# Polochon-street/bliss-rs

Hardware: AMD Instinct MI355X
Metric: songs/sec (3-min 22 050 Hz f32) at 1/2/4/8 GPU; HBM GB/s vs roofline (higher is better)
Workload: dtype f32; 1 GPU; configs[1]: batch of 1024 synthetic 3969000-sample (3-min) white-noise f32 PCM buffers per GPU, full 23-feature descriptor set (FeaturesVersion 2); songs_per_gpu=1024, songs_total=1024, features=23, parallelism=single GPU

## Files before the change

bliss-rs_amd/csrc/kernels_chroma.hip:

```cpp
#include <float.h>
#include <stdlib.h>

#include <type_traits>

#include "device_utils.hpp"
#include "fft_r16.hpp"
#include "internal.hpp"

namespace bg {

typedef double double4_t __attribute__((ext_vector_type(4)));

__device__ __forceinline__ double tuning_of_slot(int slot) {
    return slot >= N_TUNING ? 0.0 : (-50.0 + (100.0 * 0.01 * (double)slot)) / 100.0;
}

__global__ __launch_bounds__(256) void chroma_bank_kernel(double* __restrict__ bank) {
#pragma clang fp contract(off)
    const int slot = blockIdx.y;
    const int k = blockIdx.x * 256 + threadIdx.x;
    if (k >= BANK_PITCH) return;
    double* out = bank + (size_t)slot * BANK_ROWS * BANK_PITCH;
    if (k >= CBINS) {
        for (int r = 0; r < BANK_ROWS; r++) out[(size_t)r * BANK_PITCH + k] = 0.0;
        return;
    }
    const double tuning = tuning_of_slot(slot);
    const double ncf = 12.0, nc2 = 6.0;
    const double step = 22050.0 / 8192.0;
    const double a440 = 440.0 * pow(2.0, tuning / 12.0);
    auto fbin = [&](int i) { return log2((0.0 + step * (double)i) / (a440 / 16.0)) * ncf; };
    const double fb1 = fbin(1);
    const double fb = (k == 0) ? fb1 - 1.5 * ncf : fbin(k);
    const double fbn = fbin(k + 1);
    double bw = fbn - fb;
    if (bw <= 1.0) bw = 1.0;
    double w[12], l2 = 0.0;
    for (int c = 0; c < 12; c++) {
        double d = -(double)c + fb;
        d = fmod(d + nc2 + 10.0 * ncf, ncf) - nc2;
        d = d / bw;
        w[c] = exp(-0.5 * (2.0 * d) * (2.0 * d));
        l2 += w[c] * w[c];
    }
    l2 = sqrt(l2);
    if (l2 < DBL_MIN) l2 = 1.0;
    const double y = (fb / ncf - 5.0) / 2.0;
    const double g = exp(-0.5 * (y * y));
    for (int r = 0; r < BANK_ROWS; r++) {
        double v = 0.0;
        if (r < 12) v = (w[(r + 3) % 12] / l2) * g;
        out[(size_t)r * BANK_PITCH + k] = v;
    }
}

void launch_chroma_bank(double* bank, hipStream_t st) {
    hipLaunchKernelGGL(chroma_bank_kernel, dim3((BANK_PITCH + 255) / 256, N_TUNING + 1), dim3(256), 0, st, bank);
}

__device__ __forceinline__ bool pip_is_peak(float sb, float se, float sa, double ref) {
    return (sa <= se) && (sb < se) && ((double)se > ref);
}

__device__ __forceinline__ void wave_append(bool is_peak, int c, uint16_t* list, uint32_t* count) {
    const uint64_t mask = __ballot(is_peak);
    if (mask == 0) return;
    const uint32_t lane = (uint32_t)lane_id();
    uint32_t base = 0;
    if (lane == 0) base = atomicAdd(count, (uint32_t)__popcll(mask));
    base = __shfl(base, 0, WAVE);
    if (is_peak) list[base + (uint32_t)__popcll(mask & ((1ull << lane) - 1ull))] = (uint16_t)c;
}

__device__ __forceinline__ bool pip_peak_core(float sb, float se, float sa, double ref, int c, double* mag_out,
                                              double* pitch_out) {
#pragma clang fp contract(off)
    if (!(sa <= se && sb < se)) return false;
    const double before = (double)sb, elem = (double)se, after = (double)sa;
    if (!(elem > ref)) return false;
    const double avg = 0.5 * (after - before);
    double shift = 2.0 * elem - after - before;
    if (fabs(shift) < DBL_MIN) shift += 1.0;
    shift = avg / shift;
    const double pitch = ((double)c + shift) * 22050.0 / 8192.0;
    if (!(pitch > 0.0)) return false;
    *mag_out = elem + 0.5 * avg * shift;
    *pitch_out = pitch;
    return true;
}

__device__ __forceinline__ bool pip_peak_mag(float sb, float se, float sa, double ref, int c, double* mag_out) {
    double pitch;
    return pip_peak_core(sb, se, sa, ref, c, mag_out, &pitch);
}

__device__ __forceinline__ int pitch_bin(double pitch) {
#pragma clang fp contract(off)
    double x = log2(pitch / (440.0 / 16.0));
    x = 12.0 * x;
    x = x - trunc(x);
    if (x >= 0.5) x -= 1.0;
    const double q = (x - -0.5) / 0.01;
    int idx = (q > 0.0) ? (int)q : 0;
    if (idx > N_TUNING - 1) idx = N_TUNING - 1;
    return idx;
}

__device__ __forceinline__ uint32_t coarse_bin(double mag) {
    const uint32_t b = __float_as_uint((float)mag) >> COARSE_SHIFT;
    return b < (uint32_t)H1_BINS ? b : (uint32_t)H1_BINS - 1;
}

__device__ __forceinline__ float ref_floor_f32(double ref) {
    float f = (float)ref;
    if ((double)f > ref) f = __uint_as_float(__float_as_uint(f) - 1u);
    return f;
}

__device__ __forceinline__ uint32_t peak_coarse_bin(float sb, float se, float sa, double ref, int c) {
    const float avg = 0.5f * (sa - sb);
    const float den = (2.0f * se - sa) - sb;
    const float shift = avg * __builtin_amdgcn_rcpf(den);
    const uint32_t bits = __float_as_uint(se + (0.5f * avg) * shift), low = bits & COARSE_LOW_MASK;
    if (se >= 1e-30f && low >= 16u && low <= COARSE_LOW_MASK - 16u) {
        const uint32_t b = bits >> COARSE_SHIFT;
        return b < (uint32_t)H1_BINS ? b : (uint32_t)H1_BINS - 1;
    }
    double mag;
    pip_peak_mag(sb, se, sa, ref, c, &mag);
    return coarse_bin(mag);
}

constexpr float PITCH_GUARD = 0.008f, PITCH_FLAT_LIMIT = 0.00390625f;
__device__ __forceinline__ int peak_pitch_bin_f32(float sb, float se, float sa, int c) {
    const float avg = 0.5f * (sa - sb);
    const float den = (2.0f * se - sa) - sb;
    if (!(se >= 1e-30f) || den < se * PITCH_FLAT_LIMIT) return -1;
    const float shift = avg * __builtin_amdgcn_rcpf(den);
    float x = 12.0f * (__builtin_amdgcn_logf((float)c + shift) + -3.3528687f);
    x = x - truncf(x);
    if (x >= 0.5f) x -= 1.0f;
    const float q = (x + 0.5f) * 100.0f;
    const float fl = floorf(q), fr = q - fl;
    if (fr < PITCH_GUARD || fr > 1.0f - PITCH_GUARD) return -1;
    const int idx = (int)fl;
    return idx < 0 ? 0 : (idx > N_TUNING - 1 ? N_TUNING - 1 : idx);
}

__device__ __attribute__((noinline)) uint32_t coarse_bin_exact(float sb, float se, float sa, double ref, int c) {
    double mag;
    pip_peak_mag(sb, se, sa, ref, c, &mag);
    return coarse_bin(mag);
}

__device__ __forceinline__ uint32_t peak_classify(float sb, float se, float sa, double ref, int c, int* pitch_bin_out) {
    const float avg = 0.5f * (sa - sb);
    const float den = (2.0f * se - sa) - sb;
    const float shift = avg * __builtin_amdgcn_rcpf(den);
    const bool normal = se >= 1e-30f;
    int pb = -1;
    if (normal && !(den < se * PITCH_FLAT_LIMIT)) {
        float x = 12.0f * (__builtin_amdgcn_logf((float)c + shift) + -3.3528687f);
        x = x - truncf(x);
        if (x >= 0.5f) x -= 1.0f;
        const float q = (x + 0.5f) * 100.0f;
        const float fl = floorf(q), fr = q - fl;
        if (!(fr < PITCH_GUARD || fr > 1.0f - PITCH_GUARD)) {
            const int idx = (int)fl;
            pb = idx < 0 ? 0 : (idx > N_TUNING - 1 ? N_TUNING - 1 : idx);
        }
    }
    *pitch_bin_out = pb;
    const uint32_t bits = __float_as_uint(se + (0.5f * avg) * shift), low = bits & COARSE_LOW_MASK;
    if (normal && low >= 16u && low <= COARSE_LOW_MASK - 16u) {
        const uint32_t b = bits >> COARSE_SHIFT;
        return b < (uint32_t)H1_BINS ? b : (uint32_t)H1_BINS - 1;
    }
    return coarse_bin_exact(sb, se, sa, ref, c);
}

__device__ __forceinline__ uint32_t peak_record(uint32_t coarse, int pitch_bin_or_neg, int c) {
    return (coarse << 18) | ((uint32_t)(pitch_bin_or_neg + 1) << 11) | (uint32_t)c;
}

constexpr int STFT_FRAMES_PER_WG = STFT_TILE;
constexpr int STFT_GROUP = 4;
constexpr int LHIST_BINS = 512;
constexpr int EX1_PITCH = 257;
constexpr int EX2_PITCH = 272;
constexpr int STFT_LDS = 16 * EX2_PITCH;
constexpr int MAGS_TOP = 2 * 4096;

__device__ constexpr float CONST_COS32[8] = {1.0f, 0.98078528040323044f, 0.92387953251128674f, 0.83146961230254524f,
                                             0.70710678118654752f, 0.55557023301960222f, 0.38268343236508977f, 0.19509032201612827f};
__device__ constexpr float CONST_SIN32[8] = {0.0f, 0.19509032201612827f, 0.38268343236508977f, 0.55557023301960222f,
                                             0.70710678118654752f, 0.83146961230254524f, 0.92387953251128674f, 0.98078528040323044f};

typedef unsigned int u32x2_t __attribute__((ext_vector_type(2)));
typedef unsigned int u32x4_t __attribute__((ext_vector_type(4)));
__device__ __forceinline__ f2 buf_load_f2(__amdgpu_buffer_rsrc_t r, uint32_t voff, uint32_t soff) {
    const u32x2_t v = __builtin_amdgcn_raw_buffer_load_b64(r, voff, soff, 0);
    return mk(__uint_as_float(v.x), __uint_as_float(v.y));
}

__device__ __forceinline__ long reflect_index(long p, long n) {
    if (p < 0) p = -p;
    else if (p >= n) p = 2 * n - 2 - p;
    return p;
}

#ifndef TRACE
#define TRACE_DECL
#define TRACE_INIT() do {} while (0)
#define TRACE_START() do {} while (0)
#define TRACE(k) do {} while (0)
#define TRACE_FLUSH() do {} while (0)
#endif

constexpr int STFT_LDS_N = 16 * EX2_PITCH;
constexpr int EXN1_PITCH = 260;
template <bool LOADWIN, bool HALVES>
__global__ __launch_bounds__(256, (LOADWIN && HALVES) ? 5 : 4) void stft8192_kernel(const float* __restrict__ pcm,
                                                       const SongDesc* __restrict__ songs, uint32_t n_songs,
                                                       const uint32_t* __restrict__ pfx_c,
                                                       const float* __restrict__ hann,
                                                       const float2* __restrict__ tw,
                                                       float* __restrict__ spec,
                                                       float* __restrict__ frame_max, uint32_t* __restrict__ h1,
                                                       uint32_t* __restrict__ peak_rec, uint32_t* __restrict__ peak_cnt,
                                                       uint32_t n_tiles) {
    constexpr bool NARROW = HALVES;
    __shared__ __attribute__((aligned(16))) float lds_raw[NARROW ? STFT_LDS_N : 2 * STFT_LDS];
    f2* const lds = reinterpret_cast<f2*>(lds_raw);
    float* const ldsf = lds_raw;
    constexpr int MAGS_TOP_W = NARROW ? 4096 : MAGS_TOP;
    __shared__ float red[4];
    __shared__ uint32_t lhist[LHIST_BINS];
    __shared__ uint32_t lhist_base;
    __shared__ uint16_t peak_list[PIP_MAX_PER_FRAME + 2];
    __shared__ uint32_t peak_count;
    __shared__ __attribute__((aligned(16))) f2 tw256[256];
    TRACE_DECL
    TRACE_INIT();
    {
        const float2 a = tw[32 * (((threadIdx.x >> 4) * (threadIdx.x & 15)) & 255)];
        tw256[threadIdx.x] = mk(a.x, a.y);
    }
    const uint32_t bx = blockIdx.x;
    const uint32_t wg = (bx & ~31u) | ((bx & 7u) << 2) | ((bx >> 3) & 3u);
    if (wg >= n_tiles) return;
    const uint32_t s = find_segment(pfx_c, n_songs, wg);
    const SongDesc sd = songs[s];
    const uint32_t tile = wg - pfx_c[s];
    const uint32_t f_first = (tile >> 2) * (uint32_t)(STFT_GROUP * STFT_FRAMES_PER_WG) + (tile & 3u);
    const float* __restrict__ x = pcm + sd.pcm_off;
    const int t = threadIdx.x;
    const long n = (long)sd.n;
    const int lo4 = t & 15, hi4 = t >> 4;

    const __amdgpu_buffer_rsrc_t r_hann = __builtin_amdgcn_make_buffer_rsrc((void*)hann, 0, W8192 * 4, 0x00020000);


    const uint32_t t8 = 8u * (uint32_t)t;
    f2 win[16];
    if constexpr (!LOADWIN) {
#pragma unroll
        for (int n1 = 0; n1 < 16; n1++) win[n1] = buf_load_f2(r_hann, t8, 2048u * n1);
    }
    f2 c_p2, c_sp;
    {
        const float2 a = tw[2 * hi4 * lo4], b = tw[t];
        c_p2 = mk(a.x, a.y);
        c_sp = mk(b.x, b.y);
        asm volatile("" : "+v"(c_p2), "+v"(c_sp));
    }
    uint32_t* hist = h1 + (size_t)s * H1_BINS;
    for (int i = t; i < LHIST_BINS; i += 256) lhist[i] = 0;
    bool have_base = false;
    __syncthreads();

    auto tw_at = [&](int m, int k) -> f2 {
        typedef float f4 __attribute__((ext_vector_type(4)));
        const f4 pair = reinterpret_cast<const f4*>(tw256)[8 * m + (k >> 1)];
        return (k & 1) ? mk(pair.z, pair.w) : mk(pair.x, pair.y);
    };
    auto load_window = [&]() {
        if constexpr (LOADWIN) {
#pragma unroll
            for (int n1 = 0; n1 < 16; n1++) win[n1] = buf_load_f2(r_hann, t8, 2048u * n1);
        }
    };
    auto load_frame = [&](uint32_t f, f2 (&xr)[16]) {
        const long w0 = (long)f * HOP_C - W8192 / 2;
        if (w0 + W8192 / 2 > n) {
#pragma unroll
            for (int n1 = 0; n1 < 16; n1++) xr[n1] = mk(0.0f, 0.0f);
        } else if (w0 >= 0 && w0 + W8192 <= n) {
            const __amdgpu_buffer_rsrc_t r_x = __builtin_amdgcn_make_buffer_rsrc((void*)(x + w0), 0, W8192 * 4, 0x00020000);
#pragma unroll
            for (int n1 = 0; n1 < 16; n1++) xr[n1] = buf_load_f2(r_x, t8, 2048u * n1);
        } else {
            const int before = w0 < 0 ? (int)(-w0) : 0;
            const long rel_l = n - w0;
            const int rel = rel_l > 0x3fffffffL ? 0x3fffffff : (int)rel_l;
            const float* __restrict__ xw = x + w0;
#pragma unroll
            for (int n1 = 0; n1 < 16; n1++) {
                int q0 = 2 * (256 * n1 + t), q1 = q0 + 1;
                q0 = q0 < before ? 2 * before - q0 : (q0 >= rel ? 2 * rel - 2 - q0 : q0);
                q1 = q1 < before ? 2 * before - q1 : (q1 >= rel ? 2 * rel - 2 - q1 : q1);
                xr[n1] = mk(xw[q0], xw[q1]);
            }
        }
    };

    f2 v[16];
    if (f_first < sd.n_c) {
        load_frame(f_first, v);
        load_window();
#pragma unroll
        for (int n1 = 0; n1 < 16; n1++) v[n1] = v[n1] * win[n1];
    }
    TRACE_START();
#pragma unroll 1
    for (int fi = 0; fi < STFT_FRAMES_PER_WG; fi++) {
        const uint32_t f = f_first + (uint32_t)(STFT_GROUP * fi);
        if (f >= sd.n_c) break;
        radix16(v);
#pragma unroll
        for (int k1 = 1; k1 < 16; k1++)
            v[R16(k1)] = cmul_pk(v[R16(k1)], tw_at(hi4, k1));
        if constexpr (NARROW) {
            f2 u[16];
#pragma unroll
            for (int k1 = 0; k1 < 16; k1++) ldsf[k1 * EXN1_PITCH + t] = v[R16(k1)].x;
            __syncthreads();
#pragma unroll
            for (int m1 = 0; m1 < 16; m1++) u[m1].x = ldsf[lo4 * EXN1_PITCH + 16 * m1 + hi4];
            __syncthreads();
#pragma unroll
            for (int k1 = 0; k1 < 16; k1++) ldsf[k1 * EXN1_PITCH + t] = v[R16(k1)].y;
            __syncthreads();
#pragma unroll
            for (int m1 = 0; m1 < 16; m1++) u[m1].y = ldsf[lo4 * EXN1_PITCH + 16 * m1 + hi4];
#pragma unroll
            for (int m1 = 0; m1 < 16; m1++) v[m1] = u[m1];
        } else {
#pragma unroll
        for (int k1 = 0; k1 < 16; k1++) lds[k1 * EX1_PITCH + t] = v[R16(k1)];
        TRACE(0);
        __syncthreads();
        TRACE(1);
#pragma unroll
        for (int m1 = 0; m1 < 16; m1++) v[m1] = lds[lo4 * EX1_PITCH + 16 * m1 + hi4];
        }
        radix16(v);
        v[R16(0)] = cmul_pk(v[R16(0)], c_p2);
#pragma unroll
        for (int j1 = 1; j1 < 16; j1++) v[R16(j1)] = cmul_pk(v[R16(j1)], cmul_pk(tw_at(hi4, j1), c_p2));
        TRACE(2);
        __syncthreads();
        TRACE(3);
        if constexpr (NARROW) {
            f2 u[16];
#pragma unroll
            for (int j1 = 0; j1 < 16; j1++) ldsf[j1 * EX2_PITCH + t] = v[R16(j1)].x;
            __syncthreads();
#pragma unroll
            for (int m2 = 0; m2 < 16; m2++) u[m2].x = ldsf[hi4 * EX2_PITCH + 16 * m2 + lo4];
            __syncthreads();
#pragma unroll
            for (int j1 = 0; j1 < 16; j1++) ldsf[j1 * EX2_PITCH + t] = v[R16(j1)].y;
            __syncthreads();
#pragma unroll
            for (int m2 = 0; m2 < 16; m2++) u[m2].y = ldsf[hi4 * EX2_PITCH + 16 * m2 + lo4];
#pragma unroll
            for (int m2 = 0; m2 < 16; m2++) v[m2] = u[m2];
        } else {
#pragma unroll
        for (int j1 = 0; j1 < 16; j1++) lds[j1 * EX2_PITCH + t] = v[R16(j1)];
        TRACE(4);
        __syncthreads();
        TRACE(5);
#pragma unroll
        for (int m2 = 0; m2 < 16; m2++) v[m2] = lds[hi4 * EX2_PITCH + 16 * m2 + lo4];
        }
        radix16(v);
        TRACE(6);
        __syncthreads();
        TRACE(7);
        constexpr int ZOFF = NARROW ? 2048 : 0;
#pragma unroll
        for (int j2 = 8; j2 < 16; j2++) lds[t + 256 * j2 - ZOFF] = v[R16(j2)];
        TRACE(8);
        __syncthreads();
        TRACE(9);
        float m_lo[8], m_hi[8], m_mid = 0.0f;
        float mx = 0.0f;
#pragma unroll
        for (int j = 0; j < 8; j++) {
            const float CJ = CONST_COS32[j], SJ = CONST_SIN32[j];
            const int k = t + 256 * j;
            float sq_k, sq_m;
            const f2 w = j == 0 ? c_sp : cmul_pk_s(c_sp, mk(CJ, -SJ));
            const f2 zm = lds[(k == 0 ? 2048 : 4096 - k) - ZOFF];
            split_pair_sq(v[R16(j)], (j == 0 && t == 0) ? v[R16(0)] : zm, w, sq_k, sq_m);
            m_lo[j] = mag_from_sq(sq_k);
            m_hi[j] = mag_from_sq(sq_m);
            mx = fmaxf(mx, fmaxf(m_lo[j], m_hi[j]));
        }
        if (t == 0) {
            m_mid = mag_from_sq(split_one_sq(v[R16(8)], v[R16(8)], mk(0.0f, -1.0f)));
            mx = fmaxf(mx, m_mid);
        }
        const bool has_next = fi + 1 < STFT_FRAMES_PER_WG && f + STFT_GROUP < sd.n_c;
        if (has_next) load_frame(f + STFT_GROUP, v);
        mx = wave_max_dpp(mx);
        if constexpr (NARROW) __syncthreads();
        float* mags = reinterpret_cast<float*>(lds);
        float* mags_top = mags + MAGS_TOP_W - 4096;
#pragma unroll
        for (int j = 0; j < 8; j++) {
            mags[t + 256 * j] = m_lo[j];
            if (j == 0 && t == 0) mags_top[4096] = m_hi[0];
            else mags[4096 - (t + 256 * j)] = m_hi[j];
        }
        if (t == 0) mags[2048] = m_mid;
        if (t >= 1 && t < CBINS_PAD - 4096) mags_top[4096 + t] = 0.0f;
        {
            int slot = t >> 6;
            asm volatile("" : "+v"(slot));
            if (lane_id() == 0) red[slot] = mx;
        }
        if (t == 0) peak_count = 0;
        TRACE(10);
        __syncthreads();
        TRACE(11);
        auto store_row = [&]() {
            const __amdgpu_buffer_rsrc_t r_row = __builtin_amdgcn_make_buffer_rsrc(
                (void*)(spec + (sd.c_off + f) * (size_t)CBINS_PAD), 0, CBINS_PAD * 4, 0x00020000);
            const u32x4_t* mags4 = reinterpret_cast<const u32x4_t*>(lds);
#pragma unroll
            for (int i = 0; i < 5; i++) {
                const int q = t + 256 * i;
                if (i < 4 || q < CBINS_PAD / 4) {
                    const u32x4_t val = i < 4 ? mags4[q] : mags4[q - 1024 + MAGS_TOP_W / 4];
                    __builtin_amdgcn_raw_buffer_store_b128(val, r_row, 16u * (uint32_t)q, 0, 2);
                }
            }
        };
        store_row();
        mx = fmaxf(fmaxf(red[0], red[1]), fmaxf(red[2], red[3]));
        if (t == 0) frame_max[sd.c_off + f] = mx;
        if (!have_base) {
            if (t == 0) {
                const uint32_t top = coarse_bin((double)mx);
                lhist_base = top > (uint32_t)(LHIST_BINS * 3 / 4) ? top - (uint32_t)(LHIST_BINS * 3 / 4) : 0u;
            }
            have_base = true;
            __syncthreads();
        }
        TRACE(12);
        const uint32_t lbase = lhist_base;
        __builtin_amdgcn_s_setprio(2);
        const double ref = 0.1 * (double)mx;
        const float thr = ref_floor_f32(ref);
        {
            uint32_t hits = 0;
#pragma unroll
            for (int h = 0; h < 2; h++) {
                float sb3[3], se3[3], sa3[3];
#pragma unroll
                for (int q = 0; q < 3; q++) {
                    const int c = t + 256 * (3 * h + q);
                    sb3[q] = mags[c > 0 ? c - 1 : 0];
                    se3[q] = mags[c];
                    sa3[q] = mags[c + 1];
                }
#pragma unroll
                for (int q = 0; q < 3; q++) {
                    const int j = 3 * h + q, c = t + 256 * j;
                    const uint32_t in_range = (256 * j >= PIP_LO && 256 * j + 255 <= PIP_HI) ? 1u : (uint32_t)(c >= PIP_LO) & (uint32_t)(c <= PIP_HI);
                    const uint32_t pk = in_range & (uint32_t)(sa3[q] <= se3[q]) & (uint32_t)(sb3[q] < se3[q]) & (uint32_t)(se3[q] > thr);
                    hits |= pk << j;
                }
            }
            const uint32_t mine = (uint32_t)__popc(hits);
            const uint32_t incl = wave_scan_incl_u32_dpp(mine);
            uint32_t wbase = 0;
            if (lane_id() == 63) wbase = atomicAdd(&peak_count, incl);
            uint32_t pos = (uint32_t)__builtin_amdgcn_readlane((int)wbase, 63) + incl - mine;
#pragma unroll
            for (int j = 0; j < 6; j++)
                if ((hits >> j) & 1u) peak_list[pos++] = (uint16_t)(t + 256 * j);
            TRACE(13);
            __syncthreads();
            TRACE(14);
            const uint32_t n_peaks = peak_count;
            uint32_t* __restrict__ recs = peak_rec + (sd.c_off + f) * (size_t)PIP_MAX_PER_FRAME;
            if (t == 0) peak_cnt[sd.c_off + f] = n_peaks;
            int c_next = t < n_peaks ? (int)peak_list[t] : PIP_LO;
            for (uint32_t i = t; i < n_peaks; i += 256) {
                const int c = c_next;
                const float sb = mags[c - 1], se = mags[c], sa = mags[c + 1];
                c_next = i + 256 < n_peaks ? (int)peak_list[i + 256] : PIP_LO;
                int pb;
                const uint32_t b = peak_classify(sb, se, sa, ref, c, &pb), rel = b - lbase;
                recs[i] = peak_record(b, pb, c);
                if (rel < (uint32_t)LHIST_BINS) atomicAdd(&lhist[rel], 1u);
                else atomicAdd(&hist[b], 1u);
            }
        }
        __builtin_amdgcn_s_setprio(0);
        if (has_next) {
            load_window();
#pragma unroll
            for (int n1 = 0; n1 < 16; n1++) v[n1] = v[n1] * win[n1];
        }
        TRACE(15);
        __syncthreads();
        TRACE(16);
    }
    TRACE_FLUSH();
    if (have_base) {
        const uint32_t lbase = lhist_base;
        for (int i = t; i < LHIST_BINS; i += 256) {
            const uint32_t c = lhist[i];
            if (c) atomicAdd(&hist[lbase + i], c);
        }
    }
}

void launch_stft8192(const Batch& b, const Workspace& w, const DeviceTables& t, hipStream_t st, int shape) {
    if (b.tiles_c == 0) return;
    auto k = stft8192_kernel<false, false>;
    if (shape == 1) k = stft8192_kernel<true, true>;
    else if (shape == 2) k = stft8192_kernel<true, false>;
    else if (shape == 3) k = stft8192_kernel<false, true>;
    hipLaunchKernelGGL(k, dim3((b.tiles_c + 31u) & ~31u), dim3(256), 0, st,
                       b.pcm, b.songs, b.n_songs, b.pfx_c, t.hann8192, t.tw8192, w.spec, w.frame_max, w.h1, w.peak_rec, w.peak_cnt,
                       b.tiles_c);
}

__global__ __launch_bounds__(256) void tune_select_kernel(const SongDesc* __restrict__ songs,
                                                          const uint32_t* __restrict__ h1,
                                                          TuningState* __restrict__ tuning,
                                                          uint32_t* __restrict__ cand_cursor, uint32_t cand_pool,
                                                          uint32_t first_song) {
    __shared__ uint32_t wsum[4];
    __shared__ uint32_t s_total, s_blo, s_bhi;
    const uint32_t s = blockIdx.x + first_song;
    const int tid = threadIdx.x;
    TuningState* ts = tuning + s;
    auto no_peaks = [&]() {
        if (tid == 0) {
            ts->n_peaks = 0; ts->tuning_idx = -1; ts->n_cand = 0; ts->b_lo = 1; ts->b_hi = 0; ts->below = 0;
            ts->cand_off = 0; ts->cand_cap = 0;
        }
    };
    if (!songs[s].ok) { no_peaks(); return; }
    const uint32_t* hist = h1 + (size_t)s * H1_BINS;
    constexpr int PER = H1_BINS / 256;
    uint32_t local[PER], sum = 0;
#pragma unroll
    for (int i = 0; i < PER; i++) { local[i] = hist[tid * PER + i]; sum += local[i]; }
    const uint32_t incl = wave_scan_incl_u32(sum);
    if (lane_id() == 63) wsum[wave_id()] = incl;
    __syncthreads();
    uint32_t base = 0;
    for (int w = 0; w < wave_id(); w++) base += wsum[w];
    if (tid == 255) s_total = base + incl;
    __syncthreads();
    const uint32_t total = s_total;
    uint32_t before = base + incl - sum;
    if (total == 0) { no_peaks(); return; }
    const uint32_t r_lo = (total - 1) / 2, r_hi = total - 1 - r_lo;
    if (tid == 0) { ts->n_peaks = total; ts->n_cand = 0; ts->tuning_idx = -1; }
#pragma unroll
    for (int i = 0; i < PER; i++) {
        const uint32_t c = local[i];
        if (c) {
            if (before <= r_lo && r_lo < before + c) { ts->b_lo = tid * PER + i; ts->below = before; s_blo = tid * PER + i; }
            if (before <= r_hi && r_hi < before + c) { ts->b_hi = tid * PER + i; s_bhi = tid * PER + i; }
        }
        before += c;
    }
    __syncthreads();
    const uint32_t blo = s_blo, bhi = s_bhi;
    uint32_t mine = 0;
#pragma unroll
    for (int i = 0; i < PER; i++) {
        const uint32_t bin = tid * PER + i;
        if (bin >= blo && bin <= bhi) mine += local[i];
    }
    mine = wave_sum(mine);
    if (lane_id() == 0) wsum[wave_id()] = mine;
    __syncthreads();
    if (tid == 0) {
        const uint32_t want = wsum[0] + wsum[1] + wsum[2] + wsum[3];
        const uint32_t off = atomicAdd(cand_cursor, want);
        if (off <= cand_pool && want <= cand_pool - off) {
            ts->cand_off = off;
            ts->cand_cap = want;
        } else {
            atomicSub(cand_cursor, want);
            ts->cand_off = 0;
            ts->cand_cap = 0;
        }
    }
}

void launch_tune_select(const Batch& b, const Workspace& w, hipStream_t st, const SongRange* r) {
    const uint32_t s0 = r ? r->s0 : 0, s1 = r ? r->s1 : b.n_songs;
    if (s1 <= s0) return;
    hipLaunchKernelGGL(tune_select_kernel, dim3(s1 - s0), dim3(256), 0, st, b.songs, w.h1, w.tuning, w.cand_cursor,
                       w.cand_cap, s0);
}

constexpr int P2_SLOW_CAP = 1024;
constexpr int P2_FRAMES_PER_WAVE = CH_TILE / 4;

__global__ __launch_bounds__(256) void tune_pass2_kernel(const SongDesc* __restrict__ songs, uint32_t n_songs,
                                                         const uint32_t* __restrict__ pfx_ct,
                                                         const float* __restrict__ spec,
                                                         const float* __restrict__ frame_max,
                                                         const uint32_t* __restrict__ peak_rec,
                                                         const uint32_t* __restrict__ peak_cnt,
                                                         TuningState* __restrict__ tuning,
                                                         uint32_t* __restrict__ hist100,
                                                         double* __restrict__ cand_mag,
                                                         uint8_t* __restrict__ cand_pb, uint32_t first_tile) {
    __shared__ uint32_t hist[N_TUNING];
    __shared__ uint32_t slow_list[4][P2_SLOW_CAP];
    const uint32_t bx = blockIdx.x + first_tile;
    const uint32_t s = find_segment(pfx_ct, n_songs, bx);
    const SongDesc sd = songs[s];
    const uint32_t tile = bx - pfx_ct[s];
    const int tid = threadIdx.x, lane = lane_id(), wave = wave_id();
    TuningState* ts = tuning + s;
    const uint32_t b_lo = ts->b_lo, b_hi = ts->b_hi;
    if (ts->n_peaks == 0) return;
    const uint32_t cand_off = ts->cand_off;
    const uint32_t cand_cap = ts->cand_cap;
    const bool pooled = cand_cap != 0;
    if (tid < N_TUNING) hist[tid] = 0;
    __syncthreads();
    uint32_t n_slow = 0;

    auto flush = [&]() {
        for (uint32_t i = lane; i < n_slow; i += WAVE) {
            const uint32_t e = slow_list[wave][i];
            const int c = (int)(e & 0xFFFFu);
            const uint32_t f = tile * CH_TILE + wave + 4 * (e >> 16);
            const float* row = spec + (sd.c_off + f) * (size_t)CBINS_PAD;
            const double ref = 0.1 * (double)frame_max[sd.c_off + f];
            double mag, pitch;
            if (pip_peak_core(row[c - 1], row[c], row[c + 1], ref, c, &mag, &pitch)) {
                const uint32_t b = coarse_bin(mag);
                if (b > b_hi) {
                    atomicAdd(&hist[pitch_bin(pitch)], 1u);
                } else if (b >= b_lo) {
                    const uint32_t slot = atomicAdd(&ts->n_cand, 1u);
                    if (pooled && slot < cand_cap) {
                        cand_mag[cand_off + slot] = mag;
                        cand_pb[cand_off + slot] = (uint8_t)pitch_bin(pitch);
                    }
                }
            }
        }
        __builtin_amdgcn_wave_barrier();
        n_slow = 0;
    };
    uint32_t n_rec_next = 0;
    {
        const uint32_t f0 = tile * CH_TILE + wave;
        if (f0 < sd.n_c) n_rec_next = peak_cnt[sd.c_off + f0];
    }
    for (int i = 0; i < P2_FRAMES_PER_WAVE; i++) {
        const uint32_t f = tile * CH_TILE + wave + 4 * i;
        if (f >= sd.n_c) break;
        const uint32_t n_rec = n_rec_next < (uint32_t)PIP_MAX_PER_FRAME ? n_rec_next : (uint32_t)PIP_MAX_PER_FRAME;
        if (i + 1 < P2_FRAMES_PER_WAVE && f + 4 < sd.n_c) n_rec_next = peak_cnt[sd.c_off + f + 4];
        const uint32_t* __restrict__ recs = peak_rec + (sd.c_off + f) * (size_t)PIP_MAX_PER_FRAME;
        if (n_slow + PIP_MAX_PER_FRAME > P2_SLOW_CAP) flush();
        for (uint32_t j0 = 0; j0 < n_rec; j0 += 4 * WAVE) {
            uint32_t r4[4];
#pragma unroll
            for (int u = 0; u < 4; u++) {
                const uint32_t j = j0 + WAVE * u + lane;
                r4[u] = j < n_rec ? recs[j] : 0xFFFFFFFFu;
            }
#pragma unroll
            for (int u = 0; u < 4; u++) {
                if (j0 + WAVE * u >= n_rec) break;
                const uint32_t j = j0 + WAVE * u + lane;
                bool slow = false;
                uint32_t c = 0;
                if (j < n_rec) {
                    const uint32_t r = r4[u];
                    const uint32_t b = r >> 18, pbf = (r >> 11) & 0x7Fu;
                    c = r & 0x7FFu;
                    if (b > b_hi) {
                        if (pbf) atomicAdd(&hist[pbf - 1], 1u);
                        else slow = true;
                    } else if (b >= b_lo) {
                        slow = true;
                    }
                }
                const uint64_t mask = __ballot(slow);
                if (mask) {
                    if (slow) slow_list[wave][n_slow + (uint32_t)__popcll(mask & ((1ull << lane) - 1ull))] = ((uint32_t)i << 16) | c;
                    n_slow += (uint32_t)__popcll(mask);
                }
            }
        }
    }
    __builtin_amdgcn_wave_barrier();
    flush();
    __syncthreads();
    if (tid < N_TUNING && hist[tid]) atomicAdd(&hist100[(size_t)s * N_TUNING + tid], hist[tid]);
}

void launch_tune_pass2(const Batch& b, const Workspace& w, hipStream_t st, const SongRange* r) {
    const uint32_t t0 = r ? r->ct0 : 0, t1 = r ? r->ct1 : b.tiles_ct;
    if (t1 <= t0) return;
    hipLaunchKernelGGL(tune_pass2_kernel, dim3(t1 - t0), dim3(256), 0, st, b.songs, b.n_songs, b.pfx_ct, w.spec,
                       w.frame_max, w.peak_rec, w.peak_cnt, w.tuning, w.hist100, w.cand_mag, w.cand_pb, t0);
}

template <typename ForEach>
__device__ uint64_t block_radix_select(ForEach&& for_each, uint32_t rank, uint32_t* hist, uint32_t* s_digit, uint32_t* s_rank,
                                       uint32_t* s_wave) {
    const int tid = threadIdx.x;
    uint64_t prefix = 0, mask = 0;
    for (int shift = 56; shift >= 0; shift -= 8) {
        hist[tid] = 0;
        __syncthreads();
        for_each([&](double mag, int) {
            const uint64_t k = f64_key(mag);
            const bool in = (k & mask) == prefix;
            const uint32_t d = (uint32_t)(k >> shift) & 0xFFu;
            const uint64_t m = __ballot(in);
            if (m != 0) {
                const int first = __ffsll((unsigned long long)m) - 1;
                const uint32_t d0 = (uint32_t)__shfl((int)d, first, WAVE);
                if (__ballot(in && d == d0) == m) {
                    if (lane_id() == first) atomicAdd(&hist[d0], (uint32_t)__popcll(m));
                } else if (in) {
                    atomicAdd(&hist[d], 1u);
                }
            }
        });
        __syncthreads();
        {
            const uint32_t h = hist[tid];
            const uint32_t incl = wave_scan_incl_u32(h);
            if (lane_id() == 63) s_wave[wave_id()] = incl;
            __syncthreads();
            uint32_t below = incl - h;
            for (int w = 0; w < wave_id(); w++) below += s_wave[w];
            if (h != 0 && below <= rank && rank < below + h) {
                *s_digit = (uint32_t)tid;
                *s_rank = rank - below;
            }
        }
        __syncthreads();
        prefix |= (uint64_t)(*s_digit) << shift;
        mask |= 0xFFull << shift;
        rank = *s_rank;
        __syncthreads();
    }
    return prefix;
}

__global__ __launch_bounds__(256) void tune_final_kernel(const SongDesc* __restrict__ songs,
                                                         TuningState* __restrict__ tuning,
                                                         const uint32_t* __restrict__ hist100,
                                                         const double* __restrict__ cand_mag,
                                                         const uint8_t* __restrict__ cand_pb,
                                                         const float* __restrict__ spec,
                                                         const float* __restrict__ frame_max,
                                                         const uint32_t* __restrict__ peak_rec,
                                                         const uint32_t* __restrict__ peak_cnt, uint32_t first_song) {
    __shared__ uint32_t hist[256];
    __shared__ uint32_t s_digit, s_rank, s_cnt_le, s_wave[4];
    __shared__ unsigned long long s_min_gt;
    const uint32_t s = blockIdx.x + first_song;
    const int tid = threadIdx.x;
    TuningState* ts = tuning + s;
    const SongDesc sd = songs[s];
    if (!sd.ok || ts->n_peaks == 0) return;
    const uint32_t total = ts->n_peaks, nc = ts->n_cand;
    const uint32_t r_lo = (total - 1) / 2, r_hi = total - 1 - r_lo;
    const uint32_t k_lo = r_lo - ts->below, k_hi = r_hi - ts->below;
    const uint32_t b_lo = ts->b_lo, b_hi = ts->b_hi;
    const bool pooled = ts->cand_cap != 0 && nc == ts->cand_cap;
    const double* v = cand_mag + ts->cand_off;
    const uint8_t* pb = cand_pb + ts->cand_off;

    auto for_each = [&](auto&& fn) {
        if (pooled) {
            for (uint32_t i0 = tid; i0 < nc; i0 += 8 * 256) {
                double m8[8];
                int b8[8];
#pragma unroll
                for (int u = 0; u < 8; u++) {
                    const uint32_t i = i0 + 256u * u;
                    m8[u] = i < nc ? v[i] : 0.0;
                    b8[u] = i < nc ? (int)pb[i] : 0;
                }
#pragma unroll
                for (int u = 0; u < 8; u++)
                    if (i0 + 256u * u < nc) fn(m8[u], b8[u]);
            }
        } else {
            for (uint32_t f = 0; f < sd.n_c; f++) {
                const uint32_t n_rec_raw = peak_cnt[sd.c_off + f];
                const uint32_t n_rec = n_rec_raw < (uint32_t)PIP_MAX_PER_FRAME ? n_rec_raw : (uint32_t)PIP_MAX_PER_FRAME;
                const uint32_t* __restrict__ recs = peak_rec + (sd.c_off + f) * (size_t)PIP_MAX_PER_FRAME;
                const float* __restrict__ row = spec + (sd.c_off + f) * (size_t)CBINS_PAD;
                const double ref = 0.1 * (double)frame_max[sd.c_off + f];
                for (uint32_t j = tid; j < n_rec; j += 256) {
                    const uint32_t r = recs[j], b = r >> 18;
                    if (b < b_lo || b > b_hi) continue;
                    const int c = (int)(r & 0x7FFu);
                    double mag, pitch;
                    if (pip_peak_core(row[c - 1], row[c], row[c + 1], ref, c, &mag, &pitch)) fn(mag, pitch_bin(pitch));
                }
            }
        }
    };

    const uint64_t key_lo = block_radix_select(for_each, k_lo, hist, &s_digit, &s_rank, s_wave);
    uint64_t key_hi = key_lo;
    if (k_hi != k_lo) {
        if (tid == 0) { s_cnt_le = 0; s_min_gt = ~0ull; }
        __syncthreads();
        uint32_t cnt = 0;
        unsigned long long mn = ~0ull;
        for_each([&](double mag, int) {
            const uint64_t k = f64_key(mag);
            if (k <= key_lo) cnt++;
            else if (k < mn) mn = k;
        });
        atomicAdd(&s_cnt_le, cnt);
        atomicMin(&s_min_gt, mn);
        __syncthreads();
        if (s_cnt_le <= k_hi) key_hi = s_min_gt;
    }
    double thr;
    {
#pragma clang fp contract(off)
        const double lo = key_f64(key_lo), hi = key_f64(key_hi);
        thr = lo + (hi - lo) / 2.0;
    }
    __syncthreads();
    if (tid < N_TUNING) hist[tid] = hist100[(size_t)s * N_TUNING + tid];
    __syncthreads();
    for_each([&](double mag, int bin) {
        if (mag >= thr) atomicAdd(&hist[bin], 1u);
    });
    __syncthreads();
    if (tid == 0) {
        uint32_t best = 0;
        for (uint32_t k = 1; k < N_TUNING; k++)
            if (hist[k] > hist[best]) best = k;
        ts->tuning_idx = (int32_t)best;
    }
}

void launch_tune_final(const Batch& b, const Workspace& w, hipStream_t st, const SongRange* r) {
    const uint32_t s0 = r ? r->s0 : 0, s1 = r ? r->s1 : b.n_songs;
    if (s1 <= s0) return;
    hipLaunchKernelGGL(tune_final_kernel, dim3(s1 - s0), dim3(256), 0, st, b.songs, w.tuning, w.hist100,
                       w.cand_mag, w.cand_pb, w.spec, w.frame_max, w.peak_rec, w.peak_cnt, s0);
}

static constexpr int TMPL_LEN[10] = {2, 2, 2, 2, 2, 2, 3, 3, 3, 3};
static constexpr int TMPL_PC[10][3] = {{0, 1, 0}, {0, 2, 0}, {0, 3, 0}, {0, 4, 0}, {0, 5, 0},
                                       {0, 6, 0}, {0, 4, 7}, {0, 3, 7}, {0, 3, 6}, {0, 4, 8}};

template <int T>
__device__ __forceinline__ double interval_feature(const double (&c)[12]) {
    double acc = 0.0;
#pragma unroll
    for (int shift = 0; shift < 12; shift++) {
        const int r0 = (TMPL_PC[T][0] + shift) % 12, r1 = (TMPL_PC[T][1] + shift) % 12;
        if (TMPL_LEN[T] == 2) {
            acc += c[r0 < r1 ? r0 : r1] * c[r0 < r1 ? r1 : r0];
        } else {
            const int r2 = (TMPL_PC[T][2] + shift) % 12;
            const int lo = r0 < r1 ? (r0 < r2 ? r0 : r2) : (r1 < r2 ? r1 : r2);
            const int hi = r0 > r1 ? (r0 > r2 ? r0 : r2) : (r1 > r2 ? r1 : r2);
            const int mid = r0 + r1 + r2 - lo - hi;
            acc += (c[lo] * c[mid]) * c[hi];
        }
    }
    return acc;
}

__global__ __launch_bounds__(256) void chroma_kernel(const SongDesc* __restrict__ songs, uint32_t n_songs, const uint32_t* __restrict__ pfx_cw,
                              const uint32_t* __restrict__ pfx_ct, const float* __restrict__ spec,
                              const double* __restrict__ bank, const TuningState* __restrict__ tuning,
                              double* __restrict__ chroma_part, double* __restrict__ dbg_chroma, uint32_t first_wg);

void launch_chroma(const Batch& b, const Workspace& w, const DeviceTables& t, hipStream_t st, const SongRange* r) {
    const uint32_t g0 = r ? r->cw0 : 0, g1 = r ? r->cw1 : b.tiles_cw;
    if (g1 <= g0) return;
    hipLaunchKernelGGL(chroma_kernel, dim3(g1 - g0), dim3(256), 0, st, b.songs, b.n_songs, b.pfx_cw, b.pfx_ct, w.spec,
                       t.chroma_bank, w.tuning, w.chroma_part, w.dbg_chroma, g0);
}

#ifndef BG_PROBE_REPLACES_CHROMA_KERNEL
__global__ __launch_bounds__(256) void chroma_kernel(const SongDesc* __restrict__ songs, uint32_t n_songs,
                                                     const uint32_t* __restrict__ pfx_cw,
                                                     const uint32_t* __restrict__ pfx_ct,
                                                     const float* __restrict__ spec,
                                                     const double* __restrict__ bank,
                                                     const TuningState* __restrict__ tuning,
                                                     double* __restrict__ chroma_part,
                                                     double* __restrict__ dbg_chroma, uint32_t first_wg) {
    __shared__ double tile_c[4][4][16][13];
    const uint32_t bx = blockIdx.x + first_wg;
    const uint32_t s = find_segment(pfx_cw, n_songs, bx);
    const SongDesc sd = songs[s];
    const int lane = lane_id(), wave = wave_id();
    const uint32_t tile64 = (bx - pfx_cw[s]) * 4 + wave;
    const uint32_t n_tiles = pfx_ct[s + 1] - pfx_ct[s];
    if (tile64 >= n_tiles) return;
    const int i16 = lane & 15, g = lane >> 4;
    const int tidx = tuning[s].tuning_idx;
    const int slot = (tidx < 0) ? N_TUNING : tidx;
    const uint32_t f0 = tile64 * CH_TILE;

    const double* __restrict__ arow = bank + ((size_t)slot * BANK_ROWS + (i16 < BANK_ROWS ? i16 : BANK_ROWS - 1)) * BANK_PITCH + 8 * g;
    const float* brow[4];
#pragma unroll
    for (int q = 0; q < 4; q++) {
        uint32_t fj = f0 + 16 * q + i16;
        if (fj >= sd.n_c) fj = sd.n_c - 1;
        brow[q] = spec + (sd.c_off + fj) * (size_t)CBINS_PAD + 8 * g;
    }
    double4_t acc[4][2];
#pragma unroll
    for (int q = 0; q < 4; q++) { acc[q][0] = double4_t{0.0, 0.0, 0.0, 0.0}; acc[q][1] = double4_t{0.0, 0.0, 0.0, 0.0}; }
    struct KBlock {
        double4_t a[2];
        float4 b[2][4];
    };
    auto k_load = [&](int k0, KBlock& kb) {
#pragma unroll
        for (int u = 0; u < 2; u++) kb.a[u] = *reinterpret_cast<const double4_t*>(arow + k0 + 4 * u);
#pragma unroll
        for (int q = 0; q < 4; q++)
#pragma unroll
            for (int u = 0; u < 2; u++) kb.b[u][q] = *reinterpret_cast<const float4*>(brow[q] + k0 + 4 * u);
        __builtin_amdgcn_sched_barrier(0);
    };
    auto k_mma = [&](const KBlock& kb) {
#pragma unroll
        for (int u = 0; u < 2; u++) {
#pragma unroll
            for (int q = 0; q < 4; q++) {
                const float4 v = kb.b[u][q];
                const double b0 = (double)v.x * (double)v.x, b1 = (double)v.y * (double)v.y;
                const double b2 = (double)v.z * (double)v.z, b3 = (double)v.w * (double)v.w;
                acc[q][0] = __builtin_amdgcn_mfma_f64_16x16x4f64(kb.a[u].x, b0, acc[q][0], 0, 0, 0);
                acc[q][1] = __builtin_amdgcn_mfma_f64_16x16x4f64(kb.a[u].y, b1, acc[q][1], 0, 0, 0);
                acc[q][0] = __builtin_amdgcn_mfma_f64_16x16x4f64(kb.a[u].z, b2, acc[q][0], 0, 0, 0);
                acc[q][1] = __builtin_amdgcn_mfma_f64_16x16x4f64(kb.a[u].w, b3, acc[q][1], 0, 0, 0);
            }
        }
    };
    constexpr int KBLOCKS = CBINS_PAD / 32;
    static_assert(CBINS_PAD % 32 == 0 && BANK_PITCH == CBINS_PAD && KBLOCKS % 2 == 1, "pairs of blocks and one last block");
    KBlock k0buf, k1buf;
    k_load(0, k0buf);
#pragma unroll 1
    for (int kb = 0; kb + 2 < KBLOCKS; kb += 2) {
        k_load(32 * (kb + 1), k1buf);
        k_mma(k0buf);
        k_load(32 * (kb + 2), k0buf);
        k_mma(k1buf);
    }
    k_mma(k0buf);
#pragma unroll
    for (int q = 0; q < 4; q++) {
        const double4_t cacc = acc[q][0] + acc[q][1];
#pragma unroll
        for (int r = 0; r < 3; r++) tile_c[wave][q][i16][g + 4 * r] = cacc[r];
    }
    __builtin_amdgcn_wave_barrier();
    double feat[10];
#pragma unroll
    for (int t = 0; t < 10; t++) feat[t] = 0.0;
    if (f0 + lane < sd.n_c) {
        double c[12], sum = 0.0;
#pragma unroll
        for (int k = 0; k < 12; k++) { c[k] = tile_c[wave][lane >> 4][lane & 15][k]; sum += fabs(c[k]); }
        if (sum < DBL_MIN) sum = 1.0;
        if (dbg_chroma) {
#pragma unroll
            for (int k = 0; k < 12; k++) dbg_chroma[(sd.c_off + f0 + lane) * 12 + k] = c[k] / sum;
        }
        double esum = 0.0;
#pragma unroll
        for (int k = 0; k < 12; k++) { c[k] = exp((c[k] / sum) * 15.0); esum += fabs(c[k]); }
        if (esum < 0.0001) esum = 1.0;
#pragma unroll
        for (int k = 0; k < 12; k++) c[k] /= esum;
        feat[0] = interval_feature<0>(c); feat[1] = interval_feature<1>(c);
        feat[2] = interval_feature<2>(c); feat[3] = interval_feature<3>(c);
        feat[4] = interval_feature<4>(c); feat[5] = interval_feature<5>(c);
        feat[6] = interval_feature<6>(c); feat[7] = interval_feature<7>(c);
        feat[8] = interval_feature<8>(c); feat[9] = interval_feature<9>(c);
    }
#pragma unroll
    for (int t = 0; t < 10; t++) {
        double v = feat[t];
        const double v1 = __shfl(v, (lane & 15) + 16, WAVE), v2 = __shfl(v, (lane & 15) + 32, WAVE), v3 = __shfl(v, (lane & 15) + 48, WAVE);
        v = __shfl(v, lane & 15, WAVE);
        v = ((v + v1) + v2) + v3;
#pragma unroll
        for (int off = 8; off > 0; off >>= 1) v += __shfl_xor(v, off, WAVE);
        if (lane == 0) chroma_part[(size_t)(pfx_ct[s] + tile64) * 10 + t] = v;
    }
}

#endif

}
```

Before: 27920 songs/sec.

## Load STFT frames with 128-bit buffer loads and remap thread lanes

Interior frames are now fetched with 128-bit buffer loads instead of pairs of 64-bit loads. A permlane32_swap step then puts each lane's data back in place. To make that work, a permuted logical thread index is used for the window loads, the twiddles and the edge-case loads, and the first transpose reads LDS through a matching column-slot remap. The narrow LDS pitch also changes from 260 to 261, presumably to shift bank mapping. This cuts global load instructions at the cost of extra cross-lane swaps and more complex index arithmetic, and the change relies on the swizzle being exactly undone.

```diff
diff --git a/bliss-rs_amd/csrc/kernels_chroma.hip b/bliss-rs_amd/csrc/kernels_chroma.hip
--- a/bliss-rs_amd/csrc/kernels_chroma.hip
+++ b/bliss-rs_amd/csrc/kernels_chroma.hip
@@ -218,7 +218,7 @@
 #endif
 
 constexpr int STFT_LDS_N = 16 * EX2_PITCH;
-constexpr int EXN1_PITCH = 260;
+constexpr int EXN1_PITCH = 261;
 template <bool LOADWIN, bool HALVES>
 __global__ __launch_bounds__(256, (LOADWIN && HALVES) ? 5 : 4) void stft8192_kernel(const float* __restrict__ pcm,
                                                        const SongDesc* __restrict__ songs, uint32_t n_songs,
@@ -261,7 +261,10 @@
     const __amdgpu_buffer_rsrc_t r_hann = __builtin_amdgcn_make_buffer_rsrc((void*)hann, 0, W8192 * 4, 0x00020000);
 
 
-    const uint32_t t8 = 8u * (uint32_t)t;
+    const int t_log = (t & ~63) | ((t & 31) << 1) | ((t >> 5) & 1);
+    const int hi4_log = t_log >> 4;
+    const uint32_t t8 = 8u * (uint32_t)t_log;
+    const uint32_t t16 = 2048u * (uint32_t)((t >> 5) & 1) + 16u * (uint32_t)(32 * (t >> 6) + (t & 31));
     f2 win[16];
     if constexpr (!LOADWIN) {
 #pragma unroll
@@ -290,7 +293,7 @@
             for (int n1 = 0; n1 < 16; n1++) win[n1] = buf_load_f2(r_hann, t8, 2048u * n1);
         }
     };
-    auto load_frame = [&](uint32_t f, f2 (&xr)[16]) {
+    auto load_frame = [&](uint32_t f, f2 (&xr)[16]) -> bool {
         const long w0 = (long)f * HOP_C - W8192 / 2;
         if (w0 + W8192 / 2 > n) {
 #pragma unroll
@@ -298,7 +301,12 @@
         } else if (w0 >= 0 && w0 + W8192 <= n) {
             const __amdgpu_buffer_rsrc_t r_x = __builtin_amdgcn_make_buffer_rsrc((void*)(x + w0), 0, W8192 * 4, 0x00020000);
 #pragma unroll
-            for (int n1 = 0; n1 < 16; n1++) xr[n1] = buf_load_f2(r_x, t8, 2048u * n1);
+            for (int j = 0; j < 8; j++) {
+                const u32x4_t q = __builtin_amdgcn_raw_buffer_load_b128(r_x, t16, 4096u * j, 0);
+                xr[2 * j] = mk(__uint_as_float(q.x), __uint_as_float(q.y));
+                xr[2 * j + 1] = mk(__uint_as_float(q.z), __uint_as_float(q.w));
+            }
+            return true;
         } else {
             const int before = w0 < 0 ? (int)(-w0) : 0;
             const long rel_l = n - w0;
@@ -306,18 +314,30 @@
             const float* __restrict__ xw = x + w0;
 #pragma unroll
             for (int n1 = 0; n1 < 16; n1++) {
-                int q0 = 2 * (256 * n1 + t), q1 = q0 + 1;
+                int q0 = 2 * (256 * n1 + t_log), q1 = q0 + 1;
                 q0 = q0 < before ? 2 * before - q0 : (q0 >= rel ? 2 * rel - 2 - q0 : q0);
                 q1 = q1 < before ? 2 * before - q1 : (q1 >= rel ? 2 * rel - 2 - q1 : q1);
                 xr[n1] = mk(xw[q0], xw[q1]);
             }
         }
+        return false;
     };
+    auto unswizzle_frame = [&](f2 (&xr)[16]) {
+#pragma unroll
+        for (int j = 0; j < 8; j++) {
+            const auto re = __builtin_amdgcn_permlane32_swap(__float_as_uint(xr[2 * j].x), __float_as_uint(xr[2 * j + 1].x), false, false);
+            const auto im = __builtin_amdgcn_permlane32_swap(__float_as_uint(xr[2 * j].y), __float_as_uint(xr[2 * j + 1].y), false, false);
+            xr[2 * j] = mk(__uint_as_float(re[0]), __uint_as_float(im[0]));
+            xr[2 * j + 1] = mk(__uint_as_float(re[1]), __uint_as_float(im[1]));
+        }
+    };
+    auto col_slot = [](int c) { return (c & ~63) | ((c & 1) << 5) | ((c & 63) >> 1); };
 
     f2 v[16];
     if (f_first < sd.n_c) {
-        load_frame(f_first, v);
+        const bool wide = load_frame(f_first, v);
         load_window();
+        if (wide) unswizzle_frame(v);
 #pragma unroll
         for (int n1 = 0; n1 < 16; n1++) v[n1] = v[n1] * win[n1];
     }
@@ -329,20 +349,21 @@
         radix16(v);
 #pragma unroll
         for (int k1 = 1; k1 < 16; k1++)
-            v[R16(k1)] = cmul_pk(v[R16(k1)], tw_at(hi4, k1));
+            v[R16(k1)] = cmul_pk(v[R16(k1)], tw_at(hi4_log, k1));
+        const int slot0 = col_slot(hi4);
         if constexpr (NARROW) {
             f2 u[16];
 #pragma unroll
             for (int k1 = 0; k1 < 16; k1++) ldsf[k1 * EXN1_PITCH + t] = v[R16(k1)].x;
             __syncthreads();
 #pragma unroll
-            for (int m1 = 0; m1 < 16; m1++) u[m1].x = ldsf[lo4 * EXN1_PITCH + 16 * m1 + hi4];
+            for (int m1 = 0; m1 < 16; m1++) u[m1].x = ldsf[lo4 * EXN1_PITCH + col_slot(16 * m1) + slot0];
             __syncthreads();
 #pragma unroll
             for (int k1 = 0; k1 < 16; k1++) ldsf[k1 * EXN1_PITCH + t] = v[R16(k1)].y;
             __syncthreads();
 #pragma unroll
-            for (int m1 = 0; m1 < 16; m1++) u[m1].y = ldsf[lo4 * EXN1_PITCH + 16 * m1 + hi4];
+            for (int m1 = 0; m1 < 16; m1++) u[m1].y = ldsf[lo4 * EXN1_PITCH + col_slot(16 * m1) + slot0];
 #pragma unroll
             for (int m1 = 0; m1 < 16; m1++) v[m1] = u[m1];
         } else {
@@ -352,7 +373,7 @@
         __syncthreads();
         TRACE(1);
 #pragma unroll
-        for (int m1 = 0; m1 < 16; m1++) v[m1] = lds[lo4 * EX1_PITCH + 16 * m1 + hi4];
+        for (int m1 = 0; m1 < 16; m1++) v[m1] = lds[lo4 * EX1_PITCH + col_slot(16 * m1) + slot0];
         }
         radix16(v);
         v[R16(0)] = cmul_pk(v[R16(0)], c_p2);
@@ -414,7 +435,7 @@
             mx = fmaxf(mx, m_mid);
         }
         const bool has_next = fi + 1 < STFT_FRAMES_PER_WG && f + STFT_GROUP < sd.n_c;
-        if (has_next) load_frame(f + STFT_GROUP, v);
+        const bool wide_next = has_next && load_frame(f + STFT_GROUP, v);
         mx = wave_max_dpp(mx);
         if constexpr (NARROW) __syncthreads();
         float* mags = reinterpret_cast<float*>(lds);
@@ -514,6 +535,7 @@
         __builtin_amdgcn_s_setprio(0);
         if (has_next) {
             load_window();
+            if (wide_next) unswizzle_frame(v);
 #pragma unroll
             for (int n1 = 0; n1 < 16; n1++) v[n1] = v[n1] * win[n1];
         }
```

Result: no change. 28030 songs/sec (median of 4 runs) (+0.4%).
